# MoonLab-YH/AOD_MEH_HUA

Hardware: AMD Instinct MI355X
Metric: images/sec train+HUA-score, RetinaNet-R50 VOC 512^2 (higher is better)
Workload: dtype bf16x3

## Files before the change

aod_meh_hua_amd/_C.py:

```python
import ctypes as C
import os

import torch

_HERE = os.path.dirname(os.path.abspath(__file__))
LIB_PATH = os.environ.get('AOD_HIP_LIB') or os.path.join(_HERE, 'lib', 'libaodhip.so')


class AodHipError(RuntimeError):
    pass


if not os.path.exists(LIB_PATH):
    raise ImportError(f'{LIB_PATH} is missing: run `python -m aod_meh_hua_amd.build` (hipcc, gfx950). '
                      'There is no CPU fallback for the MEH/HUA hot path.')
lib = C.CDLL(LIB_PATH)


class ConvSeg(C.Structure):
    _fields_ = [('B', C.c_int32), ('H', C.c_int32), ('W', C.c_int32), ('OH', C.c_int32), ('OW', C.c_int32),
                ('src_row0', C.c_int64), ('dst_row0', C.c_int64)]


class ConvDesc(C.Structure):
# ... 81 lines not shown
    'aod_pad_cast_colsum': (C.c_int, [P, P, P, P, I64, I32, I32, I32, P]),
    'aod_assign_ws_bytes': (SZ, [I32, I32]),
    'aod_max_iou_assign': (C.c_int, [P, P, I64, I32, P, P, P, I32, F32, F32, F32, I32, I32, P, P, P, P, P, P, P, P, P, I32, P, P]),
    'aod_loss_partials_len': (SZ, [I64]),
    'aod_edl_focal_l1_fwd': (C.c_int, [P, P, P, P, P, P, I64, I32, F32, F32, P, P, P, P]),
    'aod_edl_focal_l1_bwd': (C.c_int, [P, P, P, P, P, P, I64, I32, F32, F32, P, P, P, F32, I32, P, P, I32, I32, I32, I32, P]),
    'aod_edl_focal_elem': (C.c_int, [P, P, I64, I32, F32, F32, P, P, P]),
    'aod_meh_loss_fwd': (C.c_int, [P, P, P, I64, P, P, P]),
    'aod_meh_loss_bwd': (C.c_int, [P, P, P, I64, P, P, I32, I32, I32, P]),
    'aod_sigmoid_focal_l1_fwd': (C.c_int, [P, P, P, P, P, P, I64, I32, F32, F32, P, P, P, P]),
    'aod_sigmoid_focal_l1_bwd': (C.c_int, [P, P, P, P, P, P, I64, I32, F32, F32, P, P, P, F32, I32, P, P, I32, I32, I32, I32, P]),
    'aod_sigmoid_focal_elem': (C.c_int, [P, P, I64, I32, F32, F32, P, P, P]),
    'aod_sigmoid_focal_l1_levels_fwd': (C.c_int, [P, P, P, P, P, P, I32, P, I32, F32, F32, P, P, P, P, I32, P, P, P]),
    'aod_sigmoid_focal_l1_levels_bwd': (C.c_int, [P, P, P, P, P, P, I32, P, I32, F32, F32, P, P, P, P, P, I32, I32, I32, I32, P]),
    'aod_loss_levels_partials_len': (SZ, [I32, P]),
    'aod_edl_focal_l1_levels_fwd': (C.c_int, [P, P, P, P, P, P, I32, P, I32, F32, F32, P, P, P, P, I32, P, P, P]),
    'aod_edl_focal_l1_levels_bwd': (C.c_int, [P, P, P, P, P, P, I32, P, I32, F32, F32, P, P, P, P, P, I32, I32, I32, I32, P]),
    'aod_meh_loss_levels_fwd': (C.c_int, [P, P, P, I32, P, P, P, P]),
    'aod_meh_loss_levels_bwd': (C.c_int, [P, P, P, I32, P, P, P, I32, I32, I32, P]),
    'aod_meh_loss_fwd_ex': (C.c_int, [P, P, P, I64, I32, P, P, P]),
    'aod_meh_loss_bwd_ex': (C.c_int, [P, P, P, I64, I32, P, P, I32, I32, I32, P]),
    'aod_meh_loss_levels_fwd_ex': (C.c_int, [P, P, P, I32, P, I32, P, P, P]),
    'aod_meh_loss_levels_bwd_ex': (C.c_int, [P, P, P, I32, P, I32, P, P, I32, I32, I32, P]),
    'aod_softmax_rowmax': (C.c_int, [P, I32, I64, I32, F32, P, P, I32, P]),
    'aod_topk_stable': (C.c_int, [P, I32, I64, I32, P, I64, P]),
    'aod_pre_nms_levels': (C.c_int, [I32, P, P, P, P, P, P, I32, I32, F32, I32, I32, P, P, P, P, F32, P, P, P, P, P, P, P, I64, P]),
    'aod_gather_decode': (C.c_int, [P, P, P, P, P, I32, I64, I32, I32, I64, P, P, P, P, F32, P, P, P, P, I64, I64, I64, I32, P]),
    'aod_nms_ws_bytes': (SZ, [I32, I32, I32]),
    'aod_multiclass_nms': (C.c_int, [P, P, I32, I32, I32, F32, F32, I32, P, P, P, P, P, P]),
    'aod_eval_match': (C.c_int, [P, P, P, P, P, P, P, I32, I32, I32, P, I32, P, P]),
    'aod_coco_match': (C.c_int, [P, P, P, P, P, P, P, P, I32, I32, I32, P, I32, P, I32, P, P]),
    'aod_hua_ws_bytes': (SZ, [I32, I32]),
    'aod_hua_score': (C.c_int, [P, P, P, P, P, P, P, P, P, I32, I32, I32, I32, I32, F32, F32, F32, I32, U64, P, I32, I32, I32, P, P, I32, P, P, P]),
    'aod_hua_score_ex': (C.c_int, [P, P, P, P, P, P, P, P, P, I32, I32, I32, I32, I32, F32, F32, F32, I32, U64, P, I32, I32, I32, P, P, I32, P,
                                   I32, P, P, P, P]),
    'aod_hua_score_ex2': (C.c_int, [P, P, P, P, P, P, P, P, P, I32, I32, I32, I32, I32, F32, F32, F32, I32, U64, P, I32, I32, I32, P, P, I32, P,
                                    I32, I32, P, P, P, P]),
    'aod_maxpool_fwd': (C.c_int, [P, P, I32, I32, I32, I32, I32, I32, I32, I32, I32, P]),
    'aod_maxpool_bwd': (C.c_int, [P, P, P, I32, I32, I32, I32, I32, I32, I32, I32, I32, P]),
    'aod_l2norm_fwd': (C.c_int, [P, P, P, I64, I32, F32, P]),
    'aod_l2norm_bwd': (C.c_int, [P, P, P, P, P, I64, I32, F32, P]),
    'aod_ssd_loss_fwd': (C.c_int, [P, P, P, P, P, P, I32, I32, I32, I32, I32, F32, P, P, P, P]),
    'aod_ssd_loss_bwd': (C.c_int, [P, P, P, P, P, P, P, P, I32, I32, I32, I32, F32, P, P, P, P, P, P]),
    'aod_synth_normal_images': (C.c_int, [P, I32, I64, U64, P, P]),
    'aod_image_xform': (C.c_int, [P, P, I32, I32, I32, P, P]),
    'aod_x3_split': (C.c_int, [P, P, I64, I32, P]),
    'aod_x3_merge': (C.c_int, [P, P, I64, I32, P]),
    'aod_x3_add': (C.c_int, [P, P, P, I64, P]),
    'aod_x3_nchw_f32_to_s2d': (C.c_int, [P, P, I32, I32, I32, I32, P]),
    'aod_x3_maxpool3x3s2': (C.c_int, [P, P, I32, I32, I32, I32, P]),
    'aod_x3_upsample2x_add_to': (C.c_int, [P, P, P, I32, I32, I32, I32, I32, I32, P]),
    'aod_x3_upsample2x_add_bwd_set': (C.c_int, [P, P, I32, I32, I32, I32, I32, I32, P]),
    'aod_x3_act_bwd': (C.c_int, [P, P, P, P, I64, I32, I32, P]),
    'aod_x3_pad_cast_colsum': (C.c_int, [P, P, P, P, I64, I32, P]),
    'aod_x3_pad_cast_colsum_map': (C.c_int, [P, P, P, P, I64, I32, P, P]),
    'aod_x3_nchw_f32_to_nhwc': (C.c_int, [P, P, I32, I32, I32, I32, P]),
    'aod_x3_maxpool_fwd': (C.c_int, [P, P, I32, I32, I32, I32, I32, I32, I32, I32, I32, P]),
    'aod_x3_maxpool_bwd': (C.c_int, [P, P, P, I32, I32, I32, I32, I32, I32, I32, I32, I32, P]),
    'aod_x3_l2norm_fwd': (C.c_int, [P, P, P, I64, I32, F32, P]),
    'aod_x3_l2norm_bwd': (C.c_int, [P, P, P, P, P, I64, I32, F32, P]),
    'aod_sgd_multi': (C.c_int, [P, P, P, P, I32, F32, P, F32, F32, I32, F32, P]),
    'aod_sgd_multi_clipped': (C.c_int, [P, P, P, P, I32, F32, P, F32, F32, I32, F32, P, P]),
    'aod_grad_norm_multi': (C.c_int, [P, P, I32, F32, F32, I32, P, I64, P, P]),
    'aod_ensemble_mi_partials_len': (SZ, [I32, P, I32]),
    'aod_ensemble_mi': (C.c_int, [P, I32, I32, P, I32, I32, P, P, I64, P]),
    'aod_dropout2d_masks': (C.c_int, [P, P, I32, P, I32, I32, F32, U64, C.c_uint32, P]),
    'aod_dropout2d_apply': (C.c_int, [P, P, I64, I32, I32, I32, I32, P]),
    'aod_dropout2d_apply_multi': (C.c_int, [P, P, I64, I32, I32, P, P, P, I32, I32, P]),
    'aod_pool_descriptor': (C.c_int, [P, I32, P, P, I32, I32, I32, P, I64, P]),
    'aod_kcenter_chunk': (C.c_int, []),
    'aod_kcenter_ws_len': (SZ, [I64]),
    'aod_kcenter_greedy': (C.c_int, [P, I64, I32, P, I64, I64, P, P, P, P, P]),
    'aod_kcenter_greedy_ex': (C.c_int, [P, I64, I32, P, I64, I64, P, P, P, P, P, I32]),
    'aod_cdal_chunk': (C.c_int, []),
    'aod_cdal_ws_len': (SZ, [I32, P, I32, I32]),
    'aod_cdal_descriptor': (C.c_int, [P, I32, P, I32, I32, F32, P, I64, P, I64, P]),
    'aod_det_uncertainty': (C.c_int, [P, P, P, P, P, I32, I32, I32, I32, I32, I32, I32, F32, P, P, P, P]),
    'aod_loc_stability_max_levels': (C.c_int, []),
    'aod_pixel_noise': (C.c_int, [P, P, I32, I32, I32, I32, P, P, F32, I32, U64, P, P]),
    'aod_loc_stability': (C.c_int, [P, P, P, I32, I32, I32, F32, I32, I32, P, P, P]),
}
for _n, (_r, _a) in _SIGS.items():
    if hasattr(lib, _n):
        getattr(lib, _n).restype = _r
        getattr(lib, _n).argtypes = _a
lib.aod_last_error.restype = C.c_char_p


def ptr(t):
    if t is None:
        return None
    if not t.is_cuda:
        raise AodHipError('aod_meh_hua_amd ops need tensors on the MI355X (cuda:N); got a CPU tensor. There is no CPU fallback.')
    return C.c_void_p(t.data_ptr())


def stream():
    return C.c_void_p(torch.cuda.current_stream().cuda_stream)


def check(rc, name='aod'):
    if rc != 0:
        raise AodHipError(f'{name} failed ({rc}): {lib.aod_last_error().decode()}')


def call(name, *args):
# ... 2 lines not shown
```

aod_meh_hua_amd/csrc/x3_ops.hip:

```cpp
#include "common.h"

static inline int grid_for(long long nvec) {
  long long b = (nvec + 255) / 256;
  return (int)(b > 2048 ? 2048 : (b < 1 ? 1 : b));
}

__device__ __forceinline__ int xoct(int q) { return ((q >> 2) << 6) + ((q & 3) << 3); }

__device__ __forceinline__ void xload(const bf16_t* __restrict__ p, float (&v)[8]) {
  const bf16x8 h = *reinterpret_cast<const bf16x8*>(p), l = *reinterpret_cast<const bf16x8*>(p + 32);
#pragma unroll
  for (int j = 0; j < 8; ++j) v[j] = (float)h[j] + (float)l[j];
}
__device__ __forceinline__ void xstore(bf16_t* __restrict__ p, const float (&v)[8]) {
  bf16x8 h, l;
#pragma unroll
  for (int j = 0; j < 8; ++j) { h[j] = (bf16_t)v[j]; l[j] = (bf16_t)(v[j] - (float)h[j]); }
  *reinterpret_cast<bf16x8*>(p) = h;
  *reinterpret_cast<bf16x8*>(p + 32) = l;
}

__global__ void x3_split_kernel(const float* __restrict__ src, bf16_t* __restrict__ dst, long long M, int C, int Q) {
  const long long n = M * Q;
  for (long long i = blockIdx.x * (long long)blockDim.x + threadIdx.x; i < n; i += (long long)gridDim.x * blockDim.x) {
// ... 122 lines not shown
  const int CP = (Q >> 2) * 64;
  for (long long i = blockIdx.x * (long long)blockDim.x + threadIdx.x; i < n; i += (long long)gridDim.x * blockDim.x) {
    const int q = i % Q; long long r = i / Q;
    const long long pix = r;
    const int x = r % W; r /= W;
    const int y = r % H; const int b = r / H;
    const int sy = min((int)(((long long)y * h) / H), h - 1), sx = min((int)(((long long)x * w) / W), w - 1);
    float s[8], d[8];
    xload(src + (((long long)b * h + sy) * w + sx) * CP + xoct(q), s);
    xload(lat + pix * CP + xoct(q), d);
#pragma unroll
    for (int j = 0; j < 8; ++j) d[j] += s[j];
    xstore(dst + pix * CP + xoct(q), d);
  }
}
extern "C" int aod_x3_upsample2x_add_to(const void* top, const void* lateral, void* out, int B, int h, int w, int C, int H, int W, aod_stream_t stream) {
  AOD_CHECK_ARG(top && lateral && out && C % 64 == 0, "x3_upsample_add_to: the X-layout width must be a multiple of 64");
  hipLaunchKernelGGL(x3_upsample_add_kernel, dim3(grid_for((long long)B * H * W * (C / 16))), dim3(256), 0, (hipStream_t)stream, (const bf16_t*)top,
                     (const bf16_t*)lateral, (bf16_t*)out, B, h, w, C / 16, H, W);
  AOD_LAUNCH_CHECK();
  return 0;
}
__global__ void x3_upsample_add_bwd_kernel(const bf16_t* __restrict__ gd, bf16_t* __restrict__ gs, int B, int h, int w, int Q, int H, int W) {
  const long long n = (long long)B * h * w * Q;
  const int CP = (Q >> 2) * 64;
  for (long long i = blockIdx.x * (long long)blockDim.x + threadIdx.x; i < n; i += (long long)gridDim.x * blockDim.x) {
    const int q = i % Q; long long r = i / Q;
    const long long pix = r;
    const int sx = r % w; r /= w;
    const int sy = r % h; const int b = r / h;
    const int y0 = (int)(((long long)sy * H + h - 1) / h), y1 = min(H, (int)(((long long)(sy + 1) * H + h - 1) / h));
    const int x0 = (int)(((long long)sx * W + w - 1) / w), x1 = min(W, (int)(((long long)(sx + 1) * W + w - 1) / w));
    float a[8];
#pragma unroll
    for (int j = 0; j < 8; ++j) a[j] = 0.f;
    for (int y = y0; y < y1; ++y)
      for (int x = x0; x < x1; ++x) {
        float v[8];
        xload(gd + (((long long)b * H + y) * W + x) * CP + xoct(q), v);
#pragma unroll
        for (int j = 0; j < 8; ++j) a[j] += v[j];
      }
    xstore(gs + pix * CP + xoct(q), a);
  }
}
extern "C" int aod_x3_upsample2x_add_bwd_set(const void* g_dst, void* g_src, int B, int h, int w, int C, int H, int W, aod_stream_t stream) {
  AOD_CHECK_ARG(g_dst && g_src && C % 64 == 0, "x3_upsample_add_bwd_set: the X-layout width must be a multiple of 64");
  hipLaunchKernelGGL(x3_upsample_add_bwd_kernel, dim3(grid_for((long long)B * h * w * (C / 16))), dim3(256), 0, (hipStream_t)stream, (const bf16_t*)g_dst,
                     (bf16_t*)g_src, B, h, w, C / 16, H, W);
  AOD_LAUNCH_CHECK();
  return 0;
}

__global__ __launch_bounds__(256) void x3_act_bwd_kernel(const bf16_t* __restrict__ g, const bf16_t* __restrict__ a, bf16_t* __restrict__ dz,
                                                         float* __restrict__ colsum, long long M, int Q, int relu, int rows_per_block, float* __restrict__ cs_ws) {
  __shared__ float sb[8][256 + 8];
  const int t = threadIdx.x, cc = t & 31, rl = t >> 5;
  const int q = blockIdx.x * 32 + cc;
  const int CP = (Q >> 2) * 64;
  const long long r0 = (long long)blockIdx.y * rows_per_block, r1 = min(M, r0 + rows_per_block);
  float s[8];
#pragma unroll
  for (int j = 0; j < 8; ++j) s[j] = 0.f;
  if (q < Q) {
    const int col = xoct(q);
    for (long long m = r0 + rl; m < r1; m += 8) {
      float v[8];
      xload(g + m * CP + col, v);
      if (relu) {
        const bf16x8 av = *reinterpret_cast<const bf16x8*>(a + m * CP + col);
#pragma unroll
        for (int j = 0; j < 8; ++j) v[j] = ((float)av[j] > 0.f) ? v[j] : 0.f;
      }
#pragma unroll
      for (int j = 0; j < 8; ++j) s[j] += v[j];
      if (dz) xstore(dz + m * CP + col, v);
    }
  }
#pragma unroll
  for (int j = 0; j < 8; ++j) sb[rl][cc * 8 + j] = s[j];
  __syncthreads();
  const int n = blockIdx.x * 256 + t;
  if (colsum && n < Q * 8) {
    float b = 0.f;
#pragma unroll
    for (int r = 0; r < 8; ++r) b += sb[r][t];
    if (cs_ws) cs_ws[(long long)blockIdx.y * (Q * 8) + n] = b;
    else atomicAdd(colsum + n, b);
  }
}
extern "C" int aod_x3_act_bwd(const void* g, const void* a, void* dz, float* colsum, int64_t M, int C, int relu, aod_stream_t stream) {
  AOD_CHECK_ARG(g && C % 64 == 0 && M >= 0, "x3_act_bwd: the X-layout width must be a multiple of 64");
  AOD_CHECK_ARG(!relu || a, "x3_act_bwd: relu needs the forward output");
  if (M == 0) return 0;
  const int Q = C / 16, panels = (Q + 31) / 32;
  long long want = 2048 / panels;
  if (want < 1) want = 1;
  long long rpb = (M + want - 1) / want;
  if (rpb < 64) rpb = 64;
  rpb = (rpb + 7) / 8 * 8;
  const int gy = (int)((M + rpb - 1) / rpb);
  float* const cs_ws = colsum ? aod_det_scratch((size_t)gy * Q * 8) : nullptr;
  hipLaunchKernelGGL(x3_act_bwd_kernel, dim3(panels, gy), dim3(256), 0, (hipStream_t)stream, (const bf16_t*)g, (const bf16_t*)a,
                     (bf16_t*)dz, colsum, (long long)M, Q, relu, (int)rpb, cs_ws);
  AOD_LAUNCH_CHECK();
  if (cs_ws) return aod_colsum_finalize(cs_ws, gy, Q * 8, Q * 8, colsum, nullptr, 0, (hipStream_t)stream);
  return 0;
}

__global__ __launch_bounds__(256) void x3_pad_cast_colsum_kernel(const float* __restrict__ g, const float* __restrict__ a, bf16_t* __restrict__ dz,
                                                                 float* __restrict__ colsum, long long M, int N, int Np, int rows_per_block, int TC,
                                                                 float* __restrict__ cs_ws, unsigned char* __restrict__ map) {
  __shared__ float red[256];
  const int RP = 256 / TC;
  const int c0 = threadIdx.x % TC, rl = threadIdx.x / TC;
  const long long r0 = (long long)blockIdx.x * rows_per_block, r1 = min(M, r0 + rows_per_block);
  for (int cb = 0; cb < Np; cb += TC) {
    const int c = cb + c0;
    const int col = ((c >> 5) << 6) + (c & 31);
    float s = 0.f;
    if (c < Np) {
      for (long long m = r0 + rl; m < r1; m += RP) {
        float v = 0.f;
        if (c < N) {
          v = g[m * N + c];
          if (a && !(a[m * N + c] > 0.f)) v = 0.f;
          if (map && !(v == 0.f)) map[m >> 6] = 1;
        }
        const bf16_t h = (bf16_t)v;
        dz[m * 2 * Np + col] = h;
        dz[m * 2 * Np + col + 32] = (bf16_t)(v - (float)h);
        s += v;
      }
    }
    __syncthreads();
    red[threadIdx.x] = s;
    __syncthreads();
    if (rl == 0 && c < N) {
      float tsum = 0.f;
      for (int r = 0; r < RP; ++r) tsum += red[r * TC + c0];
      if (cs_ws) cs_ws[(long long)blockIdx.x * N + c] = tsum;
      else atomicAdd(colsum + c, tsum);
    }
  }
}
__global__ __launch_bounds__(256) void x3_pad_cast_colsum_v8_kernel(const float* __restrict__ g, const float* __restrict__ a, bf16_t* __restrict__ dz,
                                                                    float* __restrict__ colsum, long long M, int N, int Np, int rows_per_block, int TC8,
                                                                    float* __restrict__ cs_ws, unsigned char* __restrict__ map) {
  __shared__ float red[256][9];
  const int RP = 256 / TC8;
  const int c8 = threadIdx.x % TC8, rl = threadIdx.x / TC8;
  const long long r0 = (long long)blockIdx.x * rows_per_block, r1 = min(M, r0 + rows_per_block);
  const int c = c8 * 8;
  const int col = ((c >> 5) << 6) + (c & 31);
  float s[8] = {0.f, 0.f, 0.f, 0.f, 0.f, 0.f, 0.f, 0.f};
  if (c < Np) {
    const bool lo = c + 4 <= N, hi = c + 8 <= N;
    for (long long m = r0 + rl; m < r1; m += RP) {
      f32x4 v0 = {0.f, 0.f, 0.f, 0.f}, v1 = {0.f, 0.f, 0.f, 0.f};
      if (lo) v0 = *reinterpret_cast<const f32x4*>(g + m * N + c);
// ... 273 lines not shown
```

aod_meh_hua_amd/functional.py:

```python
import torch
from torch.autograd import Function

from . import hipops as ho
from .hipops import Seg


def as_rows(x):
    B, C, H, W = x.shape
    xr = x.permute(0, 2, 3, 1)
    if not xr.is_contiguous():
        xr = xr.contiguous()
    return xr.view(B * H * W, C)


def as_nchw(rows, B, H, W):
    return rows.view(B, H, W, rows.shape[1]).permute(0, 3, 1, 2)


def multi_rows(tensors):
    rows = [as_rows(t) for t in tensors]
    if len(rows) == 1:
        t = tensors[0]
        return rows[0], [Seg(t.shape[0], t.shape[2], t.shape[3], 0)]
    rb = rows[0].shape[1] * rows[0].element_size()
# ... 113 lines not shown
                self.tables.clear()
            recs = (_PrepRec * len(stale))()
            blk = 0
            for r, i in zip(recs, stale):
                it = self.order[i]
                src = [x() if x is not None else None for x in it.srcs]
                for t in src:
                    assert t is None or (t.dtype == torch.float32 and t.is_contiguous()), 'parameters must be contiguous fp32'
                r.w, r.gamma, r.beta, r.mean, r.var = (None if t is None else t.data_ptr() for t in src)
                r.wf, r.wd = it.wf.data_ptr(), (it.wd.data_ptr() if it.wd is not None else None)
                r.scale, r.shift, r.invstd = ((t.data_ptr() if t is not None else None) for t in (it.scale, it.shift, it.invstd))
                r.O, r.I, r.RS, r.Ipad, r.Opad = it.dims
                r.blk0, r.eps, r.pad_ = blk, it.eps, int(it.x3)
                blk += it.nblk
            host = torch.frombuffer(bytearray(bytes(recs)), dtype=torch.uint8)
            dev = self.order[stale[0]].wf.device
            ent = self.tables[stale] = (host.to(dev), blk)
        self.table = ent[0]
        ho.call('aod_param_prep', ho.ptr(ent[0]), len(stale), ent[1], ho.stream())
        for i in stale:
            self.order[i].ver = self._versions(self.order[i])


PREP = ParamPrep()


import os as _os
_FUSE_ACT = _os.environ.get('AOD_FUSE_ACT', '1') != '0'


_PREC = _os.environ.get('AOD_CONV_PREC', 'bf16x3')
assert _PREC in ('bf16', 'bf16x3'), f'AOD_CONV_PREC={_PREC!r}: bf16x3 (reference precision) or bf16 (fast mode)'
ho.X3 = _PREC == 'bf16x3'


def set_precision(p):
    global _PREC
    assert p in ('bf16', 'bf16x3')
    _PREC = p
    ho.X3 = p == 'bf16x3'


def x3_to_f32(x, channels=None):
    if not ho.X3 or x.dtype != torch.bfloat16:
        return x.float()
    B, Wd, H, W = x.shape
    rows = ho.x3_merge(as_rows(x), channels)
    return as_nchw(rows, B, H, W)


class ForkFn(Function):

    @staticmethod
    def forward(ctx, x, n):
        return tuple(x.view_as(x) for _ in range(n))

    @staticmethod
    def backward(ctx, *gs):
        tot = None
        for g in gs:
            if g is None:
                continue
            g = g.contiguous(memory_format=torch.channels_last)
            tot = g if tot is None else as_nchw(ho.x3_add(as_rows(tot), as_rows(g)), g.shape[0], g.shape[2], g.shape[3])
        return tot, None


def fork(x, n):
    if not ho.X3 or n == 1 or not (torch.is_grad_enabled() and x.requires_grad):
        return [x] * n
    return list(ForkFn.apply(x, n))


def get_precision():
    return _PREC


def mode_key():
    return (_PREC, bool(ho.DETERMINISTIC))


class ActSlot:
    __slots__ = ('masked', 's1', 'res_ok', 'res_grad')

    def __init__(self):
        self.masked, self.s1 = False, None
        self.res_ok, self.res_grad = False, None


class BwdChain:
    __slots__ = ('meta', 'x_rows', 'prep', 'out')

    def __init__(self):
        self.meta, self.x_rows, self.prep, self.out = {}, {}, {}, {}


def bwd_chain_for(blk, x):
    on = _os.environ.get('AOD_FUSE_BOTTLENECK_BWD', '1') != '0' and not ho.DETERMINISTIC
    if ho.X3 and _os.environ.get('AOD_FUSE_BOTTLENECK128_X3_BWD', '1') == '0':
        return None
    return BwdChain() if on and _FUSE_ACT and bottleneck128_train_applies(blk, x) else None


def set_deterministic(on=True):
    ho.set_deterministic(on)


class GradAcc:
    __slots__ = ('n', 'arrived', 'partial', 'slot', '__weakref__')

    def __init__(self, slot=None):
        self.n, self.arrived, self.partial = 0, 0, None
        self.slot = slot


_JUNCTIONS = []


def share_input_grad(x):
    if torch.is_grad_enabled() and x.requires_grad and _os.environ.get('AOD_GRAD_JUNCTIONS', '1') != '0':
        x._aod_acc = GradAcc(getattr(x, '_aod_slot', None) if _FUSE_ACT and _os.environ.get('AOD_JUNCTION_MASK', '1') != '0' else None)
        _JUNCTIONS.append(_weakref.ref(x._aod_acc))
    return x

# ... 179 lines not shown
    return gw, wdot


class ConvFn(Function):

    @staticmethod
    def forward(ctx, meta, w, gamma, beta, mean, var, bias, res, *xs):
        O, I, R, S = w.shape
        cin = xs[0].shape[1]
        x_rows, x_segs = multi_rows(xs)
        pi = PREP.get(w, (gamma, beta, mean, var) if gamma is not None else None, cin, meta['eps'])
        wp, scale, shift, invstd = pi.wf, pi.scale, pi.shift, pi.invstd
        if gamma is None and bias is not None:
            shift = bias.detach()
        res_rows = as_rows(res) if res is not None else None
        out_rows = as_rows(meta['out']) if meta.get('out') is not None else None
        if meta.get('pre') is not None:
            y_rows, y_segs = meta['pre'], ho.out_segs(x_segs, R, S, meta['stride'], meta['pad'], meta['dil'])
        else:
            r = ho.conv2d_rows(x_rows, x_segs, wp, O, R, S, meta['stride'], meta['pad'], meta['dil'], pre_scale=scale,
                               pre_shift=shift, res=res_rows, relu=meta['relu'], out_f32=meta['out_f32'], out=out_rows, alg=(I, O))
            y_rows, y_segs = r[0], r[1]
        ctx.meta, ctx.x_segs, ctx.y_segs = meta, x_segs, y_segs
        ctx.has_bn, ctx.has_bias, ctx.has_res = gamma is not None, bias is not None, res is not None
        ctx.nx = len(xs)
        ctx.scope = ho.SCOPE
        ctx.save_for_backward(w, gamma, mean, scale, invstd, x_rows, y_rows if meta['relu'] else None)
        if meta.get('chain') is not None:
            ch, role = meta['chain']
            ch.meta[role], ch.x_rows[role], ch.prep[role] = meta, x_rows, (w, gamma, mean, cin, x_segs)
        outs = tuple(as_nchw(y_rows[s.row0:s.row0 + s.rows], s.B, s.H, s.W) for s in y_segs)
        return outs

    @staticmethod
    def backward(ctx, *gouts):
        with ho.scope(ctx.scope):
            return ConvFn._backward(ctx, *gouts)

    @staticmethod
    def _backward(ctx, *gouts):
        w, gamma, mean, scale, invstd, x_rows, a_rows = ctx.saved_tensors
        meta = ctx.meta
        O, I, R, S = w.shape
        cin = x_rows.shape[1]
        y_segs = ctx.y_segs
        X = ho.X3
        Opad = ho.xw(O) if X else (O + 7) // 8 * 8
        g_rows = _grad_rows(gouts, y_segs, O if (meta['out_f32'] or not X) else Opad, w.device)
        dsegs = dense_segs(y_segs)
        need_w = ctx.needs_input_grad[1]
        need_x = any(ctx.needs_input_grad[8:])
        need_res = ctx.has_res and ctx.needs_input_grad[7]
        gw = ggamma = gbeta = gbias = gres = None
        if (meta['out_f32'] and X) or (Opad != O and not X):
            if meta.get('sparse_grad') and X and ho.sparse_bwd():
                dz, gbias_v, rmap = ho.pad_cast_colsum(g_rows, Opad, a_rows if meta['relu'] else None, want_map=True)
                _keep_map(dz, rmap)
            else:
                dz, gbias_v = ho.pad_cast_colsum(g_rows, Opad, a_rows if meta['relu'] else None)
            gm = None
        else:
            relu = meta['relu']
            slot = meta.get('slot')
            if slot is not None and slot.masked and g_rows.dtype == torch.bfloat16:
                dz, s1 = g_rows, slot.s1
                slot.masked, slot.s1 = False, None
            else:
                plain = (not relu) and g_rows.dtype == torch.bfloat16
                known = _S1_OF.pop(g_rows.data_ptr(), None) if plain and _os.environ.get('AOD_S1_REUSE', '1') != '0' else None
                if known is not None and known[1].shape == g_rows.shape:
                    dz, s1 = g_rows, known[0]
                else:
                    dz, _, s1, _ = ho.act_bwd(g_rows, a_rows, None, None, None, None, relu=relu, want_gm=False, want_dz=not plain)
                    if plain:
                        dz = g_rows
            gbias_v = s1
        need_bn = ctx.has_bn and ctx.needs_input_grad[2]
        if ctx.has_bias and ctx.needs_input_grad[6]:
            gbias = gbias_v[:O]
        if need_res:
            res_slot = meta.get('res_slot')
            if res_slot is not None:
                res_slot.res_grad = dz
            else:
                s = y_segs[0]
                gres = as_nchw(dz, s.B, s.H, s.W)
                if (Opad == O or X) and len(y_segs) == 1:
                    _WgradQueue.begin_pass()
                    _S1_OF[dz.data_ptr()] = (s1, dz)
        x_segs = ctx.x_segs
        if need_w or need_bn:
            dst = _grad_slice(w, dz.device) if need_w else None
            gw, ggamma = _wgrad(x_rows, x_segs, dz, dsegs, R, S, meta['stride'], meta['pad'], meta['dil'], (I, O), w, O, I, dst,
                                scale=scale if ctx.has_bn else None, bn=(s1, mean, invstd) if need_bn else None, gamma=gamma if need_bn else None,
                                zmap=_map_of(dz))
            if need_bn:
                gbeta = s1
            if not need_w:
                gw = None
        gxs = [None] * ctx.nx
        if need_x:
            wd = PREP.get(w, (gamma, None, mean, None) if ctx.has_bn else None, cin, meta['eps']).wd
            if ho.width(I) != cin or wd is None:
                raise RuntimeError('dgrad through a channel-padded input is not supported')
            xd = dense_segs(x_segs)
            in_slot = meta.get('in_slot')
            fuse = in_slot is not None and all(a.row0 == b.row0 for a, b in zip(x_segs, xd)) and all(ctx.needs_input_grad[8:])
            s1_in = ho.zeros_f32(I, dz.device) if fuse else None
            res_g = in_slot.res_grad if in_slot is not None else None
            if res_g is not None and not fuse:
                raise RuntimeError('a deferred residual gradient was left for a conv that cannot fuse it')
            acc = meta.get('in_acc')
            jslot = None
            if acc is not None:
                assert not fuse and len(xd) == 1
                res_g = acc.partial
                if acc.arrived == acc.n - 1 and acc.slot is not None and dz.dtype == torch.bfloat16 and xd[0].row0 == x_segs[0].row0:
# ... 38 lines not shown
                    acc.partial, acc.arrived = None, 0
        return (None, gw, ggamma, gbeta, None, None, gbias, gres) + tuple(gxs)


def _chain_ready(ch, meta3):
    if set(ch.meta) != {1, 2, 3} or ch.out:
        return False
    m1, m2 = ch.meta[1], ch.meta[2]
    sl1, sl2 = m1.get('in_slot'), m2.get('in_slot')
    if sl1 is None or sl2 is None or meta3.get('res_slot') is not sl1 or sl1.res_grad is None:
        return False
    if m1.get('in_acc') is not None or m2.get('in_acc') is not None:
        return False
    for r in (1, 2, 3):
        segs = ch.prep[r][4]
        if len(segs) != 1 or segs[0].row0 != 0:
            return False
    return True


def conv_bn_act(xs, w, bn=None, bias=None, res=None, stride=1, pad=0, dil=1, relu=False, out_f32=False, out=None, sole_consumer=False,
                shared_input=False, pre=None, chain=None, sparse_grad=False):
    single = torch.is_tensor(xs)
    xl = [xs] if single else list(xs)
    meta = dict(stride=stride, pad=pad, dil=dil, relu=relu, out_f32=out_f32, eps=bn.eps if bn is not None else 0.0, out=out, pre=pre,
                sparse_grad=bool(sparse_grad and out_f32))
    if chain is not None and torch.is_grad_enabled():
        meta['chain'] = chain
    if torch.is_grad_enabled():
        if relu and not out_f32:
            meta['slot'] = ActSlot()
        if sole_consumer and _FUSE_ACT:
            slots = [getattr(x, '_aod_slot', None) for x in xl]
            if slots[0] is not None and all(sl is slots[0] for sl in slots) and all(x.requires_grad for x in xl):
                if sole_consumer != 'res' or len(xl) == 1:
                    meta['in_slot'] = slots[0]
                    slots[0].res_ok = sole_consumer == 'res'
        if shared_input and len(xl) == 1:
            acc = getattr(xl[0], '_aod_acc', None)
            if acc is not None and 'in_slot' not in meta:
                meta['in_acc'] = acc
                acc.n += 1
        rs = getattr(res, '_aod_slot', None) if res is not None else None
        if rs is not None and rs.res_ok:
            meta['res_slot'] = rs
            rs.res_ok = False
    if bn is not None:
        outs = ConvFn.apply(meta, w, bn.weight, bn.bias, bn.running_mean, bn.running_var, None, res, *xl)
    else:
        outs = ConvFn.apply(meta, w, None, None, None, None, bias, res, *xl)
    if meta.get('slot') is not None:
        for o in outs:
            o._aod_slot = meta['slot']
    return outs[0] if single else list(outs)


class ConvPairFn(Function):

    @staticmethod
    def forward(ctx, meta, wA, bA, wB, bB, *xs):
        nl = len(xs) // 2
        O, I, R, S = wA.shape
        rows, segs = zip(multi_rows(xs[:nl]), multi_rows(xs[nl:]))
        assert segs[0] == segs[1] and wB.shape == wA.shape, 'paired tower convs need identical geometry'
        cin = rows[0].shape[1]
        pis = [PREP.get(w, None, cin, 0.0) for w in (wA, wB)]
        rows, wfs, shifts = list(rows), [pi.wf for pi in pis], [bA.detach(), bB.detach()]
        rider = meta.get('rider')
        if rider is not None:
            convL, xL = rider
            rows.append(xL)
            wfs.append(PREP.get(convL.weight, None, cin, 0.0).wf)
            shifts.append(convL.bias.detach())
        fmap = meta.get('fwd_map')
        omaps = [None, fmap] + ([fmap] if rider is not None else []) if fmap is not None else None
        if FWD_MAP_LOG is not None:
            FWD_MAP_LOG.append((len(rows), (sum(s.rows for s in segs[0]), ho.width(O)), omaps))
        outs, y_segs = ho.conv2d_rows_grouped(rows, list(segs[0]), wfs, O, R, S, 1, meta['pad'], meta['dil'], pre_shifts=shifts, relu=True,
                                              alg=(I, O), omaps=omaps)
        if rider is not None:
            meta['rider_out'] = outs[2]
        ctx.meta, ctx.x_segs, ctx.y_segs, ctx.nl = meta, list(segs[0]), y_segs, nl
        ctx.save_for_backward(wA, wB, rows[0], rows[1], outs[0], outs[1])
        return tuple(as_nchw(o[s.row0:s.row0 + s.rows], s.B, s.H, s.W) for o in outs[:2] for s in y_segs)

    @staticmethod
    def backward(ctx, *gouts):
        wA, wB, xA, xB, yA, yB = ctx.saved_tensors
        meta, nl, y_segs, x_segs = ctx.meta, ctx.nl, ctx.y_segs, ctx.x_segs
        O, I, R, S = wA.shape
        dsegs, xd = dense_segs(y_segs), dense_segs(x_segs)
        dzs, gws, gbs = [], [], []
        for gi, (w, x_rows, a_rows) in enumerate(((wA, xA, yA), (wB, xB, yB))):
            g_rows = _grad_rows(gouts[gi * nl:(gi + 1) * nl], y_segs, ho.width(O), w.device)
            slot = meta['slot'][gi]
            if slot is not None and slot.masked and g_rows.dtype == torch.bfloat16:
                dz, s1 = g_rows, slot.s1
                slot.masked, slot.s1 = False, None
            else:
                dz, _, s1, _ = ho.act_bwd(g_rows, a_rows, None, None, None, None, relu=True, want_gm=False, want_dz=True)
            dzs.append(dz)
            gbs.append(s1[:O] if ctx.needs_input_grad[2 + 2 * gi] else None)
            gw = None
            if ctx.needs_input_grad[1 + 2 * gi]:
                gw, _ = _wgrad(x_rows, x_segs, dz, dsegs, R, S, 1, meta['pad'], meta['dil'], (I, O), w, O, I, _grad_slice(w, dz.device),
                               zmap=_map_of(dz))
# ... 591 lines not shown
```

aod_meh_hua_amd/hipops.py:

```python
import ctypes as C
import os
from dataclasses import dataclass
from typing import List, Optional, Sequence

import torch

from . import _C
from ._C import ConvDesc, ConvSeg, call, lib, ptr, stream


X3 = False
DETERMINISTIC = False


def set_deterministic(on=True):
    global DETERMINISTIC
    rc = lib.aod_set_deterministic(1 if on else 0)
    if rc < 0:
        raise RuntimeError(lib.aod_last_error().decode())
    DETERMINISTIC = bool(on)


def xw(c):
    return 2 * ((c + 31) // 32 * 32)
# ... 590 lines not shown
    oh, ow = out_hw(seg.H, seg.W, 3, 3, 2, 1, 1)
    out = torch.empty(seg.B * oh * ow, Cc, dtype=torch.bfloat16, device=x_rows.device)
    call('aod_x3_maxpool3x3s2' if X3 else 'aod_maxpool3x3s2', ptr(x_rows), ptr(out), seg.B, seg.H, seg.W, Cc, stream())
    return out, Seg(seg.B, oh, ow, 0)


def upsample_add_(dst_rows, dst_seg: Seg, src_rows, src_seg: Seg):
    call('aod_upsample2x_add', ptr(src_rows), ptr(dst_rows), dst_seg.B, src_seg.H, src_seg.W, dst_rows.shape[1],
         dst_seg.H, dst_seg.W, stream())
    return dst_rows


def upsample_add(lat_rows, dst_seg: Seg, top_rows, src_seg: Seg):
    out = torch.empty_like(lat_rows)
    call('aod_x3_upsample2x_add_to' if X3 else 'aod_upsample2x_add_to', ptr(top_rows), ptr(lat_rows), ptr(out), dst_seg.B, src_seg.H, src_seg.W, lat_rows.shape[1], dst_seg.H, dst_seg.W, stream())
    return out


def upsample_add_bwd(g_dst_rows, dst_seg: Seg, src_seg: Seg):
    out = torch.empty(src_seg.rows, g_dst_rows.shape[1], dtype=torch.bfloat16, device=g_dst_rows.device)
    call('aod_x3_upsample2x_add_bwd_set' if X3 else 'aod_upsample2x_add_bwd_set', ptr(g_dst_rows), ptr(out), dst_seg.B, src_seg.H, src_seg.W, g_dst_rows.shape[1], dst_seg.H, dst_seg.W, stream())
    return out


def upsample_add_bwd_(g_src_rows, src_seg: Seg, g_dst_rows, dst_seg: Seg):
    call('aod_upsample2x_add_bwd', ptr(g_dst_rows), ptr(g_src_rows), dst_seg.B, src_seg.H, src_seg.W,
         g_dst_rows.shape[1], dst_seg.H, dst_seg.W, stream())
    return g_src_rows


def add_relu(a, b):
    out = torch.empty_like(a)
    call('aod_add_relu', ptr(a), ptr(b), ptr(out), a.numel(), stream())
    return out


def act_bwd(g, a=None, z=None, scale=None, mean=None, invstd=None, relu=True, want_gm=False, want_dz=True):
    M, N = g.shape
    if X3:
        assert z is None and scale is None and not want_gm and g.dtype == torch.bfloat16
        dz = torch.empty(M, N, dtype=torch.bfloat16, device=g.device) if want_dz else None
        dbeta = zeros_f32(N // 2, g.device)
        call('aod_x3_act_bwd', ptr(g), ptr(a), ptr(dz), ptr(dbeta), M, N, int(relu), stream())
        return dz, None, dbeta, None
    dz = torch.empty(M, N, dtype=torch.bfloat16, device=g.device) if want_dz else None
    gm = torch.empty(M, N, dtype=torch.bfloat16, device=g.device) if want_gm else None
    dbeta = zeros_f32(N, g.device)
    dgamma = zeros_f32(N, g.device) if z is not None else None
    call('aod_act_bwd', ptr(g), ptr(a), ptr(z), ptr(scale), ptr(mean), ptr(invstd), ptr(dz), ptr(gm), ptr(dbeta),
         ptr(dgamma), M, N, int(relu), int(g.dtype == torch.float32), stream())
    return dz, gm, dbeta, dgamma


FOCAL_FORMS = {'edl': 'aod_edl_focal', 'sigmoid': 'aod_sigmoid_focal'}


def edl_focal_l1_fwd(cls, labels, label_w, bbox_pred=None, bbox_tgt=None, bbox_w=None, gamma=2.0, alpha=0.25, sums=None, form='edl'):
    rows, Cc = cls.shape
    loss_noR = torch.empty(rows, dtype=torch.float32, device=cls.device)
    if sums is None:
        sums = zeros_f32(3, cls.device)
    part = torch.empty(max(int(_C.lib.aod_loss_partials_len(rows)), 1), dtype=torch.float32, device=cls.device)
    prof_bytes(form + '_l1_fwd', rows * (Cc * 4 + 8 + 4 + (48 if bbox_pred is not None else 0) + 4),
               lambda: call(FOCAL_FORMS[form] + '_l1_fwd', ptr(cls), ptr(labels), ptr(label_w), ptr(bbox_pred), ptr(bbox_tgt), ptr(bbox_w), rows, Cc,
                            gamma, alpha, ptr(loss_noR), ptr(sums), ptr(part), stream()))
    return loss_noR, sums


def edl_focal_l1_bwd(cls, labels, label_w, bbox_pred, bbox_tgt, bbox_w, g_cls, g_bbox, g_noR=None, g_noR_scalar=0.0,
                     gamma=2.0, alpha=0.25, g_noR_is_scalar=False, out_bf16=False, A=1, pitch_cls=None, pitch_box=None, grad_cls=None, grad_bbox=None,
                     form='edl'):
    rows, Cc = cls.shape
    pitch_cls = pitch_cls or A * Cc
    pitch_box = pitch_box or A * 4
    dt = torch.bfloat16 if out_bf16 else torch.float32
    alloc = lambda pitch, width: (torch.empty if pitch == width else torch.zeros)(rows // A, pitch, dtype=dt, device=cls.device)
    if grad_cls is None:
        grad_cls = alloc(pitch_cls, A * Cc)
    if grad_bbox is None and bbox_pred is not None:
        grad_bbox = alloc(pitch_box, A * 4)
    esz = 2 if out_bf16 else 4
    prof_bytes(form + '_l1_bwd', rows * (Cc * 4 + 8 + 4 + (4 if (g_noR is not None and not g_noR_is_scalar) else 0) + Cc * esz + ((48 + 4 * esz) if bbox_pred is not None else 0)),
               lambda: call(FOCAL_FORMS[form] + '_l1_bwd', ptr(cls), ptr(labels), ptr(label_w), ptr(bbox_pred), ptr(bbox_tgt), ptr(bbox_w), rows, Cc,
                            gamma, alpha, ptr(g_cls), ptr(g_bbox), ptr(g_noR), float(g_noR_scalar), int(bool(g_noR_is_scalar)), ptr(grad_cls), ptr(grad_bbox), int(out_bf16), A,
                            pitch_cls, pitch_box, stream()))
    return grad_cls, grad_bbox


MEH_FORMS = {'l2': 0, 'l1': 1, 'msle': 2}


def meh_loss_fwd(lam, loss_noR, bbox_w4, out_sum=None, form='l2'):
    n = lam.numel()
    if out_sum is None:
        out_sum = zeros_f32(1, lam.device)
    part = torch.empty(max(int(_C.lib.aod_loss_partials_len(n)), 1), dtype=torch.float32, device=lam.device)
    if form != 'l2':
        call('aod_meh_loss_fwd_ex', ptr(lam), ptr(loss_noR), ptr(bbox_w4), n, MEH_FORMS[form], ptr(out_sum), ptr(part), stream())
        return out_sum
    call('aod_meh_loss_fwd', ptr(lam), ptr(loss_noR), ptr(bbox_w4), n, ptr(out_sum), ptr(part), stream())
    return out_sum


def meh_loss_bwd(lam, loss_noR, bbox_w4, g, out_bf16=False, A=1, pitch=None, grad=None, form='l2'):
    n = lam.numel()
    pitch = pitch or A
# ... 209 lines not shown
```

include/aod_hip.h:

```cpp
#ifndef AOD_HIP_H
#define AOD_HIP_H
#include <stddef.h>
#include <stdint.h>

#ifdef __cplusplus
extern "C" {
#endif

typedef void* aod_stream_t;

const char* aod_last_error(void);
int aod_version(void);

typedef struct {
  int32_t B, H, W;
  int32_t OH, OW;
  int64_t src_row0;
  int64_t dst_row0;
} aod_conv_seg_t;

typedef struct {
  int32_t C, N;
  int32_t R, S;
  int32_t stride, pad, dil;
// ... 280 lines not shown
int aod_image_xform(const void* src_pack, const aod_image_xform_item_t* items_dev, int B, int Hp, int Wp, float* dst, aod_stream_t stream);

int aod_sgd_multi(void* const* params, void* const* grads, void* const* moms, const int64_t* sizes, int ntensors,
                  float lr, const float* lr_dev, float momentum, float weight_decay, int first_step, float grad_scale,
                  aod_stream_t stream);
int aod_sgd_multi_clipped(void* const* params, void* const* grads, void* const* moms, const int64_t* sizes, int ntensors,
                          float lr, const float* lr_dev, float momentum, float weight_decay, int first_step, float grad_scale,
                          const float* coef_dev, aod_stream_t stream);
int aod_grad_norm_multi(void* const* grads, const int64_t* sizes, int ntensors, float grad_scale, float max_norm, int flags,
                        float* partials_ws, int64_t ws_capacity, float* state, aod_stream_t stream);

size_t aod_ensemble_mi_partials_len(int L, const int64_t* n_per_level, int B);
int aod_ensemble_mi(const void* const* maps, int K, int L, const int64_t* n_per_level, int B, int n_cls, float* out, float* partials_ws,
                    int64_t ws_capacity, aod_stream_t stream);

int aod_dropout2d_masks(float* table, const int64_t* image_ids, int B, const int32_t* site_offsets, int n_sites, int T, float rate,
                        uint64_t seed, uint32_t sample, aod_stream_t stream);
int aod_dropout2d_apply(void* x, const float* table_row0, int64_t row_stride_T, int B, int HW, int C, int x3, aod_stream_t stream);
int aod_dropout2d_apply_multi(void* x, const float* table, int64_t row_stride_T, int B, int nseg, const int64_t* seg_row0,
                              const int32_t* seg_hw, const int32_t* seg_off, int C, int x3, aod_stream_t stream);

int aod_pool_descriptor(const void* base, int nseg, const int64_t* seg_row0, const int32_t* seg_hw, int C, int x3, int B, float* out,
                        int64_t out_stride, aod_stream_t stream);
int aod_kcenter_chunk(void);
size_t aod_kcenter_ws_len(int64_t N);
int aod_kcenter_greedy(const float* desc, int64_t N, int D, const int64_t* labelled, int64_t n_labelled, int64_t budget, int64_t* picks,
                       float* radius, float* mind, void* ws, aod_stream_t stream);

int aod_cdal_chunk(void);
size_t aod_cdal_ws_len(int L, const int64_t* rows_per_level, int C, int B);
int aod_cdal_descriptor(const void* const* maps, int L, const int64_t* rows_per_level, int C, int B, float score_thr, float* out,
                        int64_t out_stride, float* ws, int64_t ws_capacity, aod_stream_t stream);
int aod_kcenter_greedy_ex(const float* desc, int64_t N, int D, const int64_t* labelled, int64_t n_labelled, int64_t budget, int64_t* picks,
                          float* radius, float* mind, void* ws, aod_stream_t stream, int metric);

int aod_det_uncertainty(const float* boxes, const float* scores, const float* dets, const int64_t* labels, const int32_t* num, int B, int n,
                        int W, int max_num, int layout, int measure, int aggregate, float score_thr, float* unc, float* obj_out,
                        int32_t* missing, aod_stream_t stream);

int aod_loc_stability_max_levels(void);
int aod_pixel_noise(const float* src, float* dst, int B, int C, int Hp, int Wp, const int32_t* hw, const float* inv_std, float sigma, int level,
                    uint64_t seed, const int64_t* image_ids, aod_stream_t stream);
int aod_loc_stability(const float* dets, const int64_t* labels, const int32_t* num, int K, int B, int max_num, float score_thr, int same_class,
                      int combine, float* unc, float* stab_out, aod_stream_t stream);

int aod_x3_split(const float* src, void* dst, int64_t M, int C, aod_stream_t stream);
int aod_x3_merge(const void* src, float* dst, int64_t M, int C, aod_stream_t stream);
int aod_x3_add(const void* a, const void* b, void* out, int64_t n, aod_stream_t stream);
int aod_x3_nchw_f32_to_s2d(const float* src, void* dst, int B, int C, int H, int W, aod_stream_t stream);
int aod_x3_maxpool3x3s2(const void* src, void* dst, int B, int H, int W, int C, aod_stream_t stream);
int aod_x3_upsample2x_add_to(const void* top, const void* lateral, void* out, int B, int h, int w, int C, int H, int W, aod_stream_t stream);
int aod_x3_upsample2x_add_bwd_set(const void* g_dst, void* g_src, int B, int h, int w, int C, int H, int W, aod_stream_t stream);
int aod_x3_act_bwd(const void* g, const void* a, void* dz, float* colsum, int64_t M, int C, int relu, aod_stream_t stream);
int aod_x3_pad_cast_colsum(const float* g, const float* relu_out_f32, void* dz, float* colsum, int64_t M, int N, aod_stream_t stream);
int aod_x3_pad_cast_colsum_map(const float* g, const float* relu_out_f32, void* dz, float* colsum, int64_t M, int N, void* map,
                               aod_stream_t stream);

int aod_bottleneck64x3_fwd(const void* x, int Cin, int B, int H, int W, const void* w1, const float* s1, const float* b1, const void* w2,
                           const float* s2, const float* b2, const void* w3, const float* s3, const float* b3, const void* res, void* y,
                           aod_stream_t stream);

int aod_bottleneck64x3_ds_fwd(const void* x, int B, int H, int W, const void* w1, const float* s1, const float* b1, const void* w2,
                              const float* s2, const float* b2, const void* w3, const float* s3, const float* b3, const void* wd,
                              const float* sd, const float* bd, void* y, aod_stream_t stream);

int aod_bottleneck128x3_fwd(const void* x, int B, int H, int W, const void* w1, const float* s1, const float* b1, const void* w2,
                            const float* s2, const float* b2, const void* w3, const float* s3, const float* b3, void* y, void* t1, void* t2,
                            aod_stream_t stream);

int aod_bottleneck128x3_bwd(const void* g, int B, int H, int W, const void* wd3, const void* wd2, const void* wd1, const void* act_t2,
                            const void* act_t1, const void* act_x, void* gx, void* gt2, void* gt1, float* colsum_t2, float* colsum_t1,
                            float* colsum_x, aod_stream_t stream);

int aod_halo_conv3x3_x3_applies(const aod_conv_desc_t* desc);
int aod_halo_conv3x3_x3(const aod_conv_desc_t* desc, const void* src, const void* w_packed, void* dst, const float* pre_shift,
                        aod_stream_t stream);

int aod_mfma_clock_probe(int iters, int workgroups, void* out_u64_pairs, float* sink, aod_stream_t stream);

int aod_stem_pool_x3_fwd(const float* img, const void* w_x, const float* scale, const float* shift, void* y, int B, int C, int H, int W,
                         aod_stream_t stream);

int aod_x3_nchw_f32_to_nhwc(const float* src, void* dst, int B, int C, int H, int W, aod_stream_t stream);
int aod_x3_maxpool_fwd(const void* x, void* y, int B, int H, int W, int C, int OH, int OW, int k, int s, int p, aod_stream_t stream);
int aod_x3_maxpool_bwd(const void* x, const void* g, void* gx, int B, int H, int W, int C, int OH, int OW, int k, int s, int p, aod_stream_t stream);
int aod_x3_l2norm_fwd(const void* x, const float* w, void* y, int64_t rows, int C, float eps, aod_stream_t stream);
int aod_x3_l2norm_bwd(const void* x, const float* w, const void* g, void* gx, float* gw, int64_t rows, int C, float eps, aod_stream_t stream);

#ifdef __cplusplus
}
#endif
#endif
```

Baseline: 736.4.

## Fold fork gradient sums into the consuming conv's activation-backward kernel

When a conv output is forked to several consumers, the backward previously summed the branch gradients with separate x3_add kernels before the conv's activation backward. Now ForkFn stashes up to three branch gradients in the conv's metadata, and a templated act_bwd kernel reads and sums them in one pass while applying the relu mask and column sums. This removes the intermediate add kernels and their extra memory round trips. In exchange it adds cross-object coupling through conv metadata, with runtime errors if the fork has another consumer. The path is on by default behind an environment flag.

```diff
diff --git a/aod_meh_hua_amd/_C.py b/aod_meh_hua_amd/_C.py
--- a/aod_meh_hua_amd/_C.py
+++ b/aod_meh_hua_amd/_C.py
@@ -157,6 +157,7 @@
     'aod_x3_upsample2x_add_to': (C.c_int, [P, P, P, I32, I32, I32, I32, I32, I32, P]),
     'aod_x3_upsample2x_add_bwd_set': (C.c_int, [P, P, I32, I32, I32, I32, I32, I32, P]),
     'aod_x3_act_bwd': (C.c_int, [P, P, P, P, I64, I32, I32, P]),
+    'aod_x3_act_bwd_sum': (C.c_int, [P, I32, P, P, P, I64, I32, I32, P]),
     'aod_x3_pad_cast_colsum': (C.c_int, [P, P, P, P, I64, I32, P]),
     'aod_x3_pad_cast_colsum_map': (C.c_int, [P, P, P, P, I64, I32, P, P]),
     'aod_x3_nchw_f32_to_nhwc': (C.c_int, [P, P, I32, I32, I32, I32, P]),
diff --git a/aod_meh_hua_amd/csrc/x3_ops.hip b/aod_meh_hua_amd/csrc/x3_ops.hip
--- a/aod_meh_hua_amd/csrc/x3_ops.hip
+++ b/aod_meh_hua_amd/csrc/x3_ops.hip
@@ -198,8 +198,10 @@
   return 0;
 }
 
-__global__ __launch_bounds__(256) void x3_act_bwd_kernel(const bf16_t* __restrict__ g, const bf16_t* __restrict__ a, bf16_t* __restrict__ dz,
-                                                         float* __restrict__ colsum, long long M, int Q, int relu, int rows_per_block, float* __restrict__ cs_ws) {
+template <int NG>
+__global__ __launch_bounds__(256) void x3_act_bwd_kernel(const bf16_t* __restrict__ g, const bf16_t* __restrict__ g1, const bf16_t* __restrict__ g2,
+                                                         const bf16_t* __restrict__ a, bf16_t* __restrict__ dz, float* __restrict__ colsum, long long M, int Q,
+                                                         int relu, int rows_per_block, float* __restrict__ cs_ws) {
   __shared__ float sb[8][256 + 8];
   const int t = threadIdx.x, cc = t & 31, rl = t >> 5;
   const int q = blockIdx.x * 32 + cc;
@@ -213,6 +215,20 @@
     for (long long m = r0 + rl; m < r1; m += 8) {
       float v[8];
       xload(g + m * CP + col, v);
+      bf16x8 sh, sl;
+      if constexpr (NG > 1) {
+#pragma unroll
+        for (int k = 1; k < NG; ++k) {
+          float y[8];
+          xload((k == 1 ? g1 : g2) + m * CP + col, y);
+#pragma unroll
+          for (int j = 0; j < 8; ++j) {
+            const float x = v[j] + y[j];
+            sh[j] = (bf16_t)x; sl[j] = (bf16_t)(x - (float)sh[j]);
+            v[j] = (float)sh[j] + (float)sl[j];
+          }
+        }
+      }
       if (relu) {
         const bf16x8 av = *reinterpret_cast<const bf16x8*>(a + m * CP + col);
 #pragma unroll
@@ -220,7 +236,12 @@
       }
 #pragma unroll
       for (int j = 0; j < 8; ++j) s[j] += v[j];
-      if (dz) xstore(dz + m * CP + col, v);
+      if (dz) {
+        if (NG > 1 && !relu) {
+          *reinterpret_cast<bf16x8*>(dz + m * CP + col) = sh;
+          *reinterpret_cast<bf16x8*>(dz + m * CP + col + 32) = sl;
+        } else xstore(dz + m * CP + col, v);
+      }
     }
   }
 #pragma unroll
@@ -235,9 +256,11 @@
     else atomicAdd(colsum + n, b);
   }
 }
-extern "C" int aod_x3_act_bwd(const void* g, const void* a, void* dz, float* colsum, int64_t M, int C, int relu, aod_stream_t stream) {
-  AOD_CHECK_ARG(g && C % 64 == 0 && M >= 0, "x3_act_bwd: the X-layout width must be a multiple of 64");
+extern "C" int aod_x3_act_bwd_sum(const void* const* gs, int ng, const void* a, void* dz, float* colsum, int64_t M, int C, int relu, aod_stream_t stream) {
+  AOD_CHECK_ARG(gs && ng >= 1 && ng <= 3 && C % 64 == 0 && M >= 0, "x3_act_bwd: 1..3 gradient tensors, the X-layout width must be a multiple of 64");
+  for (int k = 0; k < ng; ++k) AOD_CHECK_ARG(gs[k], "x3_act_bwd: gradient tensor %d is null", k);
   AOD_CHECK_ARG(!relu || a, "x3_act_bwd: relu needs the forward output");
+  AOD_CHECK_ARG(ng == 1 || dz, "x3_act_bwd: the sum of several gradient tensors needs its destination");
   if (M == 0) return 0;
   const int Q = C / 16, panels = (Q + 31) / 32;
   long long want = 2048 / panels;
@@ -247,11 +270,21 @@
   rpb = (rpb + 7) / 8 * 8;
   const int gy = (int)((M + rpb - 1) / rpb);
   float* const cs_ws = colsum ? aod_det_scratch((size_t)gy * Q * 8) : nullptr;
-  hipLaunchKernelGGL(x3_act_bwd_kernel, dim3(panels, gy), dim3(256), 0, (hipStream_t)stream, (const bf16_t*)g, (const bf16_t*)a,
-                     (bf16_t*)dz, colsum, (long long)M, Q, relu, (int)rpb, cs_ws);
+  const bf16_t* const g0 = (const bf16_t*)gs[0];
+  const bf16_t* const g1 = ng > 1 ? (const bf16_t*)gs[1] : nullptr;
+  const bf16_t* const g2 = ng > 2 ? (const bf16_t*)gs[2] : nullptr;
+#define AOD_X3_ACT_BWD(NG_)                                                                                                             \
+  hipLaunchKernelGGL(x3_act_bwd_kernel<NG_>, dim3(panels, gy), dim3(256), 0, (hipStream_t)stream, g0, g1, g2, (const bf16_t*)a, (bf16_t*)dz, \
+                     colsum, (long long)M, Q, relu, (int)rpb, cs_ws)
+  if (ng == 1) AOD_X3_ACT_BWD(1); else if (ng == 2) AOD_X3_ACT_BWD(2); else AOD_X3_ACT_BWD(3);
+#undef AOD_X3_ACT_BWD
   AOD_LAUNCH_CHECK();
   if (cs_ws) return aod_colsum_finalize(cs_ws, gy, Q * 8, Q * 8, colsum, nullptr, 0, (hipStream_t)stream);
   return 0;
+}
+extern "C" int aod_x3_act_bwd(const void* g, const void* a, void* dz, float* colsum, int64_t M, int C, int relu, aod_stream_t stream) {
+  AOD_CHECK_ARG(g, "x3_act_bwd: null gradient");
+  return aod_x3_act_bwd_sum(&g, 1, a, dz, colsum, M, C, relu, stream);
 }
 
 __global__ __launch_bounds__(256) void x3_pad_cast_colsum_kernel(const float* __restrict__ g, const float* __restrict__ a, bf16_t* __restrict__ dz,
diff --git a/aod_meh_hua_amd/functional.py b/aod_meh_hua_amd/functional.py
--- a/aod_meh_hua_amd/functional.py
+++ b/aod_meh_hua_amd/functional.py
@@ -189,24 +189,28 @@
 class ForkFn(Function):
 
     @staticmethod
-    def forward(ctx, x, n):
+    def forward(ctx, x, n, conv_meta=None):
+        ctx.conv_meta = conv_meta
         return tuple(x.view_as(x) for _ in range(n))
 
     @staticmethod
     def backward(ctx, *gs):
+        live = [g.contiguous(memory_format=torch.channels_last) for g in gs if g is not None]
+        meta = ctx.conv_meta
+        if meta is not None and 2 <= len(live) <= 3 and ho.fold_junction_sums() and all(
+                g.dtype == torch.bfloat16 and g.shape == live[0].shape for g in live):
+            meta['junction'] = [as_rows(g) for g in live]
+            return live[0], None, None
         tot = None
-        for g in gs:
-            if g is None:
-                continue
-            g = g.contiguous(memory_format=torch.channels_last)
+        for g in live:
             tot = g if tot is None else as_nchw(ho.x3_add(as_rows(tot), as_rows(g)), g.shape[0], g.shape[2], g.shape[3])
-        return tot, None
+        return tot, None, None
 
 
 def fork(x, n):
     if not ho.X3 or n == 1 or not (torch.is_grad_enabled() and x.requires_grad):
         return [x] * n
-    return list(ForkFn.apply(x, n))
+    return list(ForkFn.apply(x, n, getattr(x, '_aod_conv_meta', None) if ho.fold_junction_sums() else None))
 
 
 def get_precision():
@@ -492,6 +496,10 @@
         need_x = any(ctx.needs_input_grad[8:])
         need_res = ctx.has_res and ctx.needs_input_grad[7]
         gw = ggamma = gbeta = gbias = gres = None
+        junction = meta.pop('junction', None)
+        if junction is not None and (len(gouts) != 1 or g_rows.data_ptr() != junction[0].data_ptr() or g_rows.shape != junction[0].shape
+                                     or g_rows.dtype != torch.bfloat16 or (meta['out_f32'] and X)):
+            raise RuntimeError('a folded gradient junction reached a conv backward that cannot add it (the forked tensor has another consumer)')
         if (meta['out_f32'] and X) or (Opad != O and not X):
             if meta.get('sparse_grad') and X and ho.sparse_bwd():
                 dz, gbias_v, rmap = ho.pad_cast_colsum(g_rows, Opad, a_rows if meta['relu'] else None, want_map=True)
@@ -502,7 +510,11 @@
         else:
             relu = meta['relu']
             slot = meta.get('slot')
-            if slot is not None and slot.masked and g_rows.dtype == torch.bfloat16:
+            if junction is not None:
+                if slot is not None and slot.masked:
+                    raise RuntimeError('a folded gradient junction and a fused activation backward met on one conv output')
+                dz, s1 = ho.act_bwd_sum(junction, a_rows if relu else None, relu=relu)
+            elif slot is not None and slot.masked and g_rows.dtype == torch.bfloat16:
                 dz, s1 = g_rows, slot.s1
                 slot.masked, slot.s1 = False, None
             else:
@@ -647,6 +659,8 @@
     if meta.get('slot') is not None:
         for o in outs:
             o._aod_slot = meta['slot']
+    if single and ho.X3 and not out_f32 and torch.is_grad_enabled():
+        outs[0]._aod_conv_meta = meta
     return outs[0] if single else list(outs)
 
 
diff --git a/aod_meh_hua_amd/hipops.py b/aod_meh_hua_amd/hipops.py
--- a/aod_meh_hua_amd/hipops.py
+++ b/aod_meh_hua_amd/hipops.py
@@ -666,6 +666,20 @@
     return dz, gm, dbeta, dgamma
 
 
+def fold_junction_sums():
+    return X3 and os.environ.get('AOD_FOLD_JUNCTION_SUMS', '1') != '0'
+
+
+def act_bwd_sum(gs, a=None, relu=True):
+    assert X3 and 2 <= len(gs) <= 3 and all(g.dtype == torch.bfloat16 and g.shape == gs[0].shape and g.is_contiguous() for g in gs)
+    M, N = gs[0].shape
+    dz = torch.empty(M, N, dtype=torch.bfloat16, device=gs[0].device)
+    dbeta = zeros_f32(N // 2, gs[0].device)
+    keep = (C.c_void_p * len(gs))(*[g.data_ptr() for g in gs])
+    call('aod_x3_act_bwd_sum', keep, len(gs), ptr(a), ptr(dz), ptr(dbeta), M, N, int(relu), stream())
+    return dz, dbeta
+
+
 FOCAL_FORMS = {'edl': 'aod_edl_focal', 'sigmoid': 'aod_sigmoid_focal'}
 
 
diff --git a/include/aod_hip.h b/include/aod_hip.h
--- a/include/aod_hip.h
+++ b/include/aod_hip.h
@@ -356,6 +356,7 @@
 int aod_x3_upsample2x_add_to(const void* top, const void* lateral, void* out, int B, int h, int w, int C, int H, int W, aod_stream_t stream);
 int aod_x3_upsample2x_add_bwd_set(const void* g_dst, void* g_src, int B, int h, int w, int C, int H, int W, aod_stream_t stream);
 int aod_x3_act_bwd(const void* g, const void* a, void* dz, float* colsum, int64_t M, int C, int relu, aod_stream_t stream);
+int aod_x3_act_bwd_sum(const void* const* gs, int ng, const void* a, void* dz, float* colsum, int64_t M, int C, int relu, aod_stream_t stream);
 int aod_x3_pad_cast_colsum(const float* g, const float* relu_out_f32, void* dz, float* colsum, int64_t M, int N, aod_stream_t stream);
 int aod_x3_pad_cast_colsum_map(const float* g, const float* relu_out_f32, void* dz, float* colsum, int64_t M, int N, void* map,
                                aod_stream_t stream);
```

Result: no change. 740.7 (median of 6 runs) (+0.6%).
